# chaeyeongyun/VQ_SEG

Hardware: AMD Instinct MI355X
Metric: train images/sec @512x512 vqreptunet1x1 K=512 (higher is better)
Workload: dtype bf16; 1 GPU; CPS training iteration (2 x vqreptunet1x1, ResNet-50 encoder, K=[0,0,512,512,512], v1 recipe: 6 forwards + 4 backwards + 2 Adam steps) on 512x512x3 images -- BASELINE configs[2] (the metric's configuration): vqreptunet1x1 512x512, K = 512; labelled_per_gpu=32, unlabelled_per_gpu=32, parallelism=dp1, collectives=none (one process), conv_dtype=bf16

## Files before the change

### vq_seg_amd/csrc/loss_kernels.h

```cpp
#pragma once
#include <hip/hip_runtime.h>
#include <stdint.h>

namespace vqseg {

struct ProtoArgs {
    const void* x;
    int bf16;
    const float* proto;
    const long long* labels;
    const unsigned char* keep;
    const float* conf;
    long M;
    int C, K, variant;
    float scale, cos_m, sin_m, th, mm;
    int easy_margin, use_margin;
};

constexpr int PROTO_ROWS_PER_BLOCK = 256;
long proto_blocks(long M);
hipError_t launch_proto_forward(const ProtoArgs& a, double* partial, double* loss, hipStream_t st);
hipError_t launch_proto_backward(const ProtoArgs& a, const float* g_loss, void* gx, float* gproto_partial, float* gproto,
                                 hipStream_t st);

struct DiceArgs {
    const float* logits;
    long sb, sc, sp;
    const long long* target;
    int B, C;
    long HW;
    long long ignore_index;
};
hipError_t launch_softmax_stats(const DiceArgs& a, long long* label, float* entropy, float* top, hipStream_t st);
size_t order_stats_workspace_bytes();
hipError_t launch_order_stats(const float* x, long n, long k, void* workspace, float* out2, hipStream_t st);
hipError_t launch_confusion(const DiceArgs& a, long long* out, hipStream_t st);
constexpr int DICE_PX_PER_BLOCK = 4096;
long dice_blocks(long HW);
hipError_t launch_dice_forward(const DiceArgs& a, double* partial, float* inter, float* sets, float* ce, hipStream_t st);
hipError_t launch_dice_backward(const DiceArgs& a, const float* g_inter, const float* g_sets, const float* g_ce, float* g_logits,
                                hipStream_t st);

struct CombineArgs {
    const float* inter[4]; const float* sets[4]; const float* ce[4];
    float* g_inter[4]; float* g_sets[4]; float* g_ce[4];
    int b[4];
    int n_sup, n_cps, c;
    float cps_weight, ce_weight, eps;
    const float* commit[4]; int n_commit, levels; float commit_weight;
    const double* proto[4]; int n_proto; float proto_weight;
    float* out;
// ... 5 lines not shown
```

### vq_seg_amd/csrc/loss_kernels.hip

```cpp
#include <hip/hip_runtime.h>
#include <stdint.h>

#include "loss_kernels.h"

namespace vqseg {

namespace {

typedef float f32x4 __attribute__((ext_vector_type(4)));
typedef unsigned int u32x4 __attribute__((ext_vector_type(4)));
constexpr int MAXC = 64, MAXK = 4;

template <typename T>
__device__ __forceinline__ void load_row(const T* __restrict__ x, long row, int C, float (&u)[MAXC]) {
    if constexpr (sizeof(T) == 2) {
        const u32x4* p = reinterpret_cast<const u32x4*>(x + row * C);
#pragma unroll
        for (int j = 0; j < MAXC / 8; ++j)
            if (j * 8 < C) {
                const u32x4 v = p[j];
#pragma unroll
                for (int e = 0; e < 4; ++e) {
                    u[j * 8 + 2 * e] = __builtin_bit_cast(float, v[e] << 16);
                    u[j * 8 + 2 * e + 1] = __builtin_bit_cast(float, v[e] & 0xFFFF0000u);
                }
            }
    } else {
        const f32x4* p = reinterpret_cast<const f32x4*>(x + row * C);
#pragma unroll
        for (int j = 0; j < MAXC / 4; ++j)
            if (j * 4 < C) {
                const f32x4 v = p[j];
#pragma unroll
                for (int e = 0; e < 4; ++e) u[j * 4 + e] = v[e];
            }
    }
}

__device__ __forceinline__ float phi_of(float c, const ProtoArgs& a) {
    float inner = 1.0f - c * c;
    inner = inner < 0.0f ? 0.0f : (inner > 1.0f ? 1.0f : inner);
    const float ph = c * a.cos_m - sqrtf(inner) * a.sin_m;
    return a.easy_margin ? (c > 0.0f ? ph : c) : (c > a.th ? ph : c - a.mm);
}
__device__ __forceinline__ float dphi_of(float c, const ProtoArgs& a) {
    const float inner = 1.0f - c * c;
    const float dsine = (inner > 0.0f && inner <= 1.0f) ? -c / sqrtf(inner) : 0.0f;
    const float d = a.cos_m - a.sin_m * dsine;
    return a.easy_margin ? (c > 0.0f ? d : 1.0f) : (c > a.th ? d : 1.0f);
}

struct RowTerms {
    double ll, w;
    double dcos[MAXK];
    float cosv[MAXK];
    float inv_n;
};

__device__ __forceinline__ RowTerms row_terms(const ProtoArgs& a, long row, float n2, const float (&dot)[MAXK], bool want_grad) {
    RowTerms t;
    const float n = fmaxf(sqrtf(n2), 1e-12f);
    t.inv_n = 1.0f / n;
    const int tgt = (int)a.labels[row];
    double z[MAXK], dz[MAXK], oh[MAXK];
#pragma unroll
    for (int c = 0; c < MAXK; ++c)
        if (c < a.K) {
            const float cs = dot[c] * t.inv_n;
            t.cosv[c] = cs;
            if (a.variant == 1) {
                oh[c] = (c == tgt ? 1.0 : 0.0) + 1e-6;
                if (a.use_margin) {
                    z[c] = oh[c] * (double)phi_of(cs, a) + (1.0 - oh[c]) * (double)cs;
                    dz[c] = oh[c] * (double)dphi_of(cs, a) + (1.0 - oh[c]);
                } else {
                    z[c] = (double)cs;
                    dz[c] = 1.0;
                }
            } else {
                oh[c] = c == tgt ? 1.0 : 0.0;
                if (c == tgt) {
                    const float ph = phi_of(cs, a);
                    z[c] = (double)(cs * ph);
                    dz[c] = (double)ph + (double)cs * (double)dphi_of(cs, a);
                } else {
                    z[c] = (double)cs;
                    dz[c] = 1.0;
                }
            }
            z[c] *= (double)a.scale;
            dz[c] *= (double)a.scale;
        }
    double S = 0.0, total = 0.0;
#pragma unroll
    for (int c = 0; c < MAXK; ++c)
        if (c < a.K) {
            S += z[c] * oh[c];
            total += exp(z[c]);
        }
    const double positive = exp(S);
    const double den = total + 1e-7;
    const double q = positive / den + 1e-7;
    t.ll = log(q);
    t.w = a.variant == 1 ? ((a.keep == nullptr || a.keep[row]) ? 1.0 : 0.0) : (a.conf ? (double)a.conf[row] : 1.0);
    if (want_grad) {
#pragma unroll
        for (int c = 0; c < MAXK; ++c)
            if (c < a.K) {
                const double dll_dz = (positive * oh[c] / den - positive * exp(z[c]) / (den * den)) / q;
                t.dcos[c] = dll_dz * dz[c];
            }
    }
    return t;
}

template <typename T>
__global__ __launch_bounds__(256) void proto_fwd_kernel(const ProtoArgs a, double* __restrict__ partial) {
    __shared__ float ps[MAXK * MAXC];
    __shared__ double red[256];
    for (int i = threadIdx.x; i < a.K * a.C; i += 256) ps[i] = a.proto[i];
    __syncthreads();
    const long row = (long)blockIdx.x * PROTO_ROWS_PER_BLOCK + threadIdx.x;
    double v = 0.0;
    if (row < a.M) {
        float u[MAXC];
        load_row<T>(reinterpret_cast<const T*>(a.x), row, a.C, u);
        float n2 = 0.0f, dot[MAXK] = {0.f, 0.f, 0.f, 0.f};
#pragma unroll
        for (int i = 0; i < MAXC; ++i)
            if (i < a.C) {
                n2 = __builtin_fmaf(u[i], u[i], n2);
#pragma unroll
                for (int c = 0; c < MAXK; ++c)
                    if (c < a.K) dot[c] = __builtin_fmaf(u[i], ps[c * a.C + i], dot[c]);
            }
        const RowTerms t = row_terms(a, row, n2, dot, false);
        v = t.ll * t.w;
    }
    red[threadIdx.x] = v;
    __syncthreads();
    for (int m = 128; m >= 1; m >>= 1) {
        if ((int)threadIdx.x < m) red[threadIdx.x] += red[threadIdx.x + m];
        __syncthreads();
    }
    if (threadIdx.x == 0) partial[blockIdx.x] = red[0];
}

__global__ __launch_bounds__(256) void proto_loss_final_kernel(const double* __restrict__ partial, long n_blocks, long M,
                                                               double* __restrict__ loss) {
    __shared__ double red[256];
    double s = 0.0;
    for (long i = threadIdx.x; i < n_blocks; i += 256) s += partial[i];
    red[threadIdx.x] = s;
    __syncthreads();
    for (int m = 128; m >= 1; m >>= 1) {
        if ((int)threadIdx.x < m) red[threadIdx.x] += red[threadIdx.x + m];
        __syncthreads();
    }
    if (threadIdx.x == 0) *loss = -red[0] / (double)M;
}

template <typename T>
__global__ __launch_bounds__(256) void proto_bwd_kernel(const ProtoArgs a, const float* __restrict__ g_loss, T* __restrict__ gx,
                                                        float* __restrict__ gproto_partial, int row_tiles) {
    __shared__ float ps[MAXK * MAXC];
    extern __shared__ float tile[];
    for (int i = threadIdx.x; i < a.K * a.C; i += 256) ps[i] = a.proto[i];
    __syncthreads();
    const int KC = a.K * a.C, G = 256 / KC;
    const int pair = threadIdx.x % KC, grp = threadIdx.x / KC;
    const int pc = pair / a.C, pi = pair % a.C;
    float* rs = tile;
    float* gcs = tile + 256 * (a.C + 1);
    float gacc = 0.0f;
    for (int rt = 0; rt < row_tiles; ++rt) {
    const long row = ((long)blockIdx.x * row_tiles + rt) * PROTO_ROWS_PER_BLOCK + threadIdx.x;
    float u[MAXC];
    float gc[MAXK] = {0.f, 0.f, 0.f, 0.f};
    float inv_n = 0.0f;
    float cosv[MAXK] = {0.f, 0.f, 0.f, 0.f};
    const bool live = row < a.M;
    if (live) {
        load_row<T>(reinterpret_cast<const T*>(a.x), row, a.C, u);
        float n2 = 0.0f, dot[MAXK] = {0.f, 0.f, 0.f, 0.f};
#pragma unroll
        for (int i = 0; i < MAXC; ++i)
            if (i < a.C) {
                n2 = __builtin_fmaf(u[i], u[i], n2);
#pragma unroll
                for (int c = 0; c < MAXK; ++c)
                    if (c < a.K) dot[c] = __builtin_fmaf(u[i], ps[c * a.C + i], dot[c]);
            }
        const RowTerms t = row_terms(a, row, n2, dot, true);
        const double k = -(double)g_loss[0] * t.w / (double)a.M;
        inv_n = t.inv_n;
#pragma unroll
        for (int c = 0; c < MAXK; ++c)
            if (c < a.K) {
                gc[c] = (float)(k * t.dcos[c]);
                cosv[c] = t.cosv[c];
            }
        float gs = 0.0f;
#pragma unroll
        for (int c = 0; c < MAXK; ++c)
            if (c < a.K) gs = __builtin_fmaf(gc[c], cosv[c], gs);
        T* grow = gx + row * a.C;
#pragma unroll
        for (int j = 0; j < MAXC / 8; ++j)
            if (j * 8 < a.C) {
                float o[8];
#pragma unroll
                for (int e = 0; e < 8; ++e) {
                    const int i = j * 8 + e;
                    float acc = -gs * (u[i] * inv_n);
#pragma unroll
                    for (int c = 0; c < MAXK; ++c)
                        if (c < a.K) acc = __builtin_fmaf(gc[c], ps[c * a.C + i], acc);
                    o[e] = acc * inv_n;
                }
                if constexpr (sizeof(T) == 2) {
                    u32x4 v;
#pragma unroll
                    for (int e = 0; e < 4; ++e) {
                        const __bf16 lo = (__bf16)o[2 * e], hi = (__bf16)o[2 * e + 1];
                        v[e] = (unsigned)__builtin_bit_cast(unsigned short, lo) | ((unsigned)__builtin_bit_cast(unsigned short, hi) << 16);
                    }
                    *reinterpret_cast<u32x4*>(grow + j * 8) = v;
                } else {
                    *reinterpret_cast<f32x4*>(grow + j * 8) = f32x4{o[0], o[1], o[2], o[3]};
                    *reinterpret_cast<f32x4*>(grow + j * 8 + 4) = f32x4{o[4], o[5], o[6], o[7]};
                }
            }
    }
    if (gproto_partial) {
#pragma unroll
        for (int i = 0; i < MAXC; ++i)
            if (i < a.C) rs[threadIdx.x * (a.C + 1) + i] = live ? u[i] * inv_n : 0.0f;
#pragma unroll
        for (int c = 0; c < MAXK; ++c) gcs[threadIdx.x * MAXK + c] = gc[c];
        __syncthreads();
        if (grp < G)
            for (int r = grp; r < PROTO_ROWS_PER_BLOCK; r += G) gacc = __builtin_fmaf(gcs[r * MAXK + pc], rs[r * (a.C + 1) + pi], gacc);
        __syncthreads();
    }
    }
    if (gproto_partial) {
        float* part = gcs + 256 * MAXK;
        part[threadIdx.x] = grp < G ? gacc : 0.0f;
        __syncthreads();
        if ((int)threadIdx.x < KC) {
            float s = 0.0f;
            for (int g = 0; g < G; ++g) s += part[g * KC + threadIdx.x];
            gproto_partial[(long)blockIdx.x * KC + threadIdx.x] = s;
        }
    }
}

__global__ __launch_bounds__(256) void proto_gproto_final_kernel(const float* __restrict__ partial, long n_blocks, int n,
                                                                 float* __restrict__ out) {
    __shared__ double red[256];
    const int i = blockIdx.x;
    double s = 0.0;
    for (long b = threadIdx.x; b < n_blocks; b += 256) s += (double)partial[b * n + i];
    red[threadIdx.x] = s;
    __syncthreads();
    for (int m = 128; m >= 1; m >>= 1) {
        if ((int)threadIdx.x < m) red[threadIdx.x] += red[threadIdx.x + m];
        __syncthreads();
    }
    if (threadIdx.x == 0) out[i] = (float)red[0];
}

}

long proto_blocks(long M) { return (M + PROTO_ROWS_PER_BLOCK - 1) / PROTO_ROWS_PER_BLOCK; }

hipError_t launch_proto_forward(const ProtoArgs& a, double* partial, double* loss, hipStream_t st) {
    const long nb = proto_blocks(a.M);
    if (a.bf16) hipLaunchKernelGGL(proto_fwd_kernel<__bf16>, dim3((unsigned)nb), dim3(256), 0, st, a, partial);
    else hipLaunchKernelGGL(proto_fwd_kernel<float>, dim3((unsigned)nb), dim3(256), 0, st, a, partial);
    hipLaunchKernelGGL(proto_loss_final_kernel, dim3(1), dim3(256), 0, st, partial, nb, a.M, loss);
    return hipGetLastError();
}

hipError_t launch_proto_backward(const ProtoArgs& a, const float* g_loss, void* gx, float* gproto_partial, float* gproto,
                                 hipStream_t st) {
    const bool gp = gproto_partial && gproto;
    int row_tiles = 1;
    if (gp) {
        const long want = (proto_blocks(a.M) + 2047) / 2048;
        row_tiles = (int)(want < 1 ? 1 : want);
    }
    const long nb = (proto_blocks(a.M) + row_tiles - 1) / row_tiles;
    const size_t lds = gp ? (size_t)(256 * (a.C + 1) + 256 * MAXK + 256) * sizeof(float) : 0;
    float* gpp = gp ? gproto_partial : nullptr;
    if (a.bf16) hipLaunchKernelGGL(proto_bwd_kernel<__bf16>, dim3((unsigned)nb), dim3(256), lds, st, a, g_loss, (__bf16*)gx, gpp, row_tiles);
    else hipLaunchKernelGGL(proto_bwd_kernel<float>, dim3((unsigned)nb), dim3(256), lds, st, a, g_loss, (float*)gx, gpp, row_tiles);
    if (gp) hipLaunchKernelGGL(proto_gproto_final_kernel, dim3(a.K * a.C), dim3(256), 0, st, gproto_partial, nb, a.K * a.C, gproto);
    return hipGetLastError();
}

namespace {
constexpr int DMAXC = 4;

__device__ __forceinline__ void dice_pixel(const DiceArgs& a, int b, long px, float (&p)[DMAXC], int& tgt, bool& keep, float& nll) {
    const long long t = a.target[(long)b * a.HW + px];
    keep = t != a.ignore_index;
    tgt = keep ? (int)t : 0;
    float z[DMAXC], mx = -__builtin_inff();
#pragma unroll
    for (int c = 0; c < DMAXC; ++c)
        if (c < a.C) {
            z[c] = keep ? a.logits[(long)b * a.sb + c * a.sc + px * a.sp] : 0.0f;
            mx = fmaxf(mx, z[c]);
        }
    float sum = 0.0f;
#pragma unroll
    for (int c = 0; c < DMAXC; ++c)
        if (c < a.C) {
            p[c] = expf(z[c] - mx);
            sum += p[c];
        }
    const float inv = 1.0f / sum;
    float zt = 0.0f;
#pragma unroll
    for (int c = 0; c < DMAXC; ++c)
        if (c < a.C) {
            p[c] *= inv;
            if (c == tgt) zt = z[c];
        }
// ... 423 lines not shown
```

### vq_seg_amd/csrc/nn_abi.hip

```cpp
#include <hip/hip_runtime.h>
#include <stdarg.h>
#include <stdio.h>
#include <string.h>

#include "../../include/vqseg.h"
#include "conv_kernels.h"
#include "vq_kernels.h"
#include "nn_kernels.h"
#include "loss_kernels.h"
#include <math.h>

extern "C" int vqseg_set_error(int code, const char* msg);

namespace {
int bad(const char* msg) { return vqseg_set_error(VQSEG_EINVAL, msg); }
int hipfail(hipError_t e, const char* where) {
    char buf[256];
    snprintf(buf, sizeof(buf), "%s: %s", where, hipGetErrorString(e));
    return vqseg_set_error((int)e, buf);
}
bool a16(const void* p) { return (reinterpret_cast<uintptr_t>(p) & 15u) == 0; }

int conv_rows_per_slot(int cout) { return cout >= 64 ? 64 : 32; }
}
// ... 73 lines not shown
        hipError_t e = vqseg::launch_conv(a, 0, static_cast<hipStream_t>(stream));
        return e == hipSuccess ? 0 : hipfail(e, "conv kernel (split-3)");
    }
    return conv2d_impl(x, x2, c1, w_hi, w_lo, y, nullptr, scale, shift, res, relu, n, h, w, cin, cout, kh, kw, stride, pad, reflect, 1,
                       ho, wo, precise, stream);
}

int vqseg_conv2d_affine_bits_f(const void* x, const void* w_hi, const float* scale, const float* shift, const void* res,
                               const unsigned char* res_bits, void* y, int n, int h, int w, int cin, int cout, int kh, int kw, int pad,
                               int ho, int wo, void* stream) {
    if (!scale || !shift || !res || !res_bits) return bad("conv2d_affine_bits: null pointer");
    if (!a16(res)) return bad("conv2d_affine_bits: pointers must be 16-byte aligned");
    if (cout % 8) return bad("conv2d_affine_bits: Cout must be a multiple of 8");
    return conv2d_impl(x, nullptr, cin, w_hi, nullptr, y, nullptr, scale, shift, res, 0, n, h, w, cin, cout, kh, kw, 1, pad, 0, 1, ho, wo, 0,
                       stream, res_bits);
}

int vqseg_conv_profile_begin(int capacity) {
    if (capacity <= 0 || capacity > (1 << 20)) return bad("conv_profile_begin: capacity out of range");
    hipError_t e = vqseg::conv_profile_begin(capacity);
    return e == hipSuccess ? 0 : hipfail(e, "conv_profile_begin");
}

int vqseg_conv_profile_collect(int max_records, double* flops_host, int* kind_host, float* ms_host, int* shape_host) {
    if (max_records <= 0 || !flops_host || !kind_host || !ms_host) return bad("conv_profile_collect: bad argument");
    return vqseg::conv_profile_collect(max_records, flops_host, kind_host, ms_host, shape_host);
}

int vqseg_set_option(const char* key, int value) {
    if (!key || value < 0) return bad("set_option: null key or negative value");
    int prev = vqseg::conv_set_option(key, value);
    if (prev < 0) prev = vqseg::vq_set_option(key, value);
    if (prev < 0) prev = vqseg::nn_set_option(key, value);
    return prev < 0 ? bad("set_option: unknown key") : prev;
}

size_t vqseg_conv2d_wgrad_workspace_bytes(int n, int h, int w, int cin, int ho, int wo, int cout, int kh, int kw) {
    if (n <= 0 || cin <= 0 || cout <= 0) return 0;
    vqseg::WgradArgs a{};
    a.N = n; a.H = h; a.W = w; a.Cin = cin; a.Ho = ho; a.Wo = wo; a.Cout = cout; a.KH = kh; a.KW = kw;
    return (size_t)vqseg::wgrad_slabs_max(a) * cout * kh * kw * cin * sizeof(float);
}

int vqseg_conv2d_wgrad2_f(const void* gy, const void* x, const void* x2, int n, const void* gy_b, const void* x_b, const void* x2_b,
                          int n_b, int c1, int h, int w, int cin, int ho, int wo, int cout, int kh, int kw, int stride, int pad,
                          int reflect, int precise, int cin_out, int im2col, int accumulate, void* workspace, size_t workspace_bytes,
                          float* gw, void* stream) {
    if (!gy || !x || !workspace || !gw) return bad("conv2d_wgrad: null pointer");
    if (n <= 0 || n_b < 0) return bad("conv2d_wgrad: bad image count");
    if (n_b > 0 && (!gy_b || !x_b)) return bad("conv2d_wgrad: second source missing");
    const int epc = precise ? 4 : 8;
    if (cin % epc || cout % epc) return bad("conv2d_wgrad: Cin and Cout must be multiples of 4 (f32) / 8 (bf16)");
    if (c1 <= 0 || c1 > cin || (c1 < cin && (!x2 || (n_b > 0 && !x2_b) || c1 % epc || (cin - c1) % epc))) return bad("conv2d_wgrad: bad channel split");
    vqseg::WgradArgs a;
    const int kkh = im2col ? 1 : kh, kkw = im2col ? 1 : kw;
    a.gy = gy; a.x = x; a.x2 = x2; a.C1 = c1; a.partial = static_cast<float*>(workspace);
    a.gy_b = gy_b; a.x_b = x_b; a.x2_b = x2_b; a.Na = n;
    a.N = n + n_b; a.H = h; a.W = w; a.Cin = cin; a.Ho = ho; a.Wo = wo; a.Cout = cout; a.KH = kkh; a.KW = kkw;
    a.stride = stride; a.pad = pad; a.reflect = reflect; a.per_tap_only = im2col;
    const int slabs = vqseg::wgrad_slabs(a, precise);
    if (workspace_bytes < (size_t)slabs * cout * kkh * kkw * cin * sizeof(float)) return vqseg_set_error(VQSEG_ENOSPC, "conv2d_wgrad: workspace too small");
    hipStream_t st = static_cast<hipStream_t>(stream);
    int final_layout = 0;
    hipError_t e = vqseg::launch_wgrad(a, precise, slabs, &final_layout, st);
    if (e != hipSuccess) return hipfail(e, "conv_wgrad_kernel");
    if (final_layout && (cin_out != cin || im2col)) return bad("conv2d_wgrad: internal layout mismatch");
// ... 412 lines not shown
```

### vq_seg_amd/csrc/nn_kernels.hip

```cpp
#include <hip/hip_runtime.h>
#include <limits.h>
#include <stdint.h>
#include <string.h>

#include "nn_kernels.h"
#include "options.h"

namespace vqseg {

typedef float f32x4 __attribute__((ext_vector_type(4)));

template <typename T>
__device__ __forceinline__ float ld(const T* p, long i) { return (float)p[i]; }
template <typename T>
__device__ __forceinline__ void st(T* p, long i, float v) { p[i] = (T)v; }

template <typename T>
struct VecN { static constexpr int N = 16 / sizeof(T); };
typedef unsigned int u32x4 __attribute__((ext_vector_type(4)));

template <typename T>
__device__ __forceinline__ void ldv(const T* p, long i, float (&v)[VecN<T>::N]) {
    const u32x4 raw = *reinterpret_cast<const u32x4*>(p + i);
    if constexpr (sizeof(T) == 4) {
// ... 734 lines not shown
    i0 = (int)s;
    if (i0 > in - 1) i0 = in - 1;
    i1 = i0 + (i0 < in - 1 ? 1 : 0);
    l1 = s - (float)i0;
}

template <typename T, int VC>
__global__ __launch_bounds__(256) void bilinear_fwd_kernel(const T* __restrict__ x, int N, int H, int W, int C, int Ho, int Wo,
                                                           int align, T* __restrict__ y) {
    constexpr int V = VecN<T>::N;
    const int cv = C / VC;
    const long total = (long)N * Ho * Wo * cv;
    for (long i = (long)blockIdx.x * 256 + threadIdx.x; i < total; i += (long)gridDim.x * 256) {
        int c, ow, oh, n;
        split_nhwc(i, cv, Wo, Ho, c, ow, oh, n);
        c *= VC;
        int h0, h1, w0, w1;
        float lh, lw;
        bil_src(oh, H, Ho, align, h0, h1, lh);
        bil_src(ow, W, Wo, align, w0, w1, lw);
        const long b = (long)n * H;
        float v00[V], v01[V], v10[V], v11[V], o[V];
        ldc<T, VC>(x, ((b + h0) * W + w0) * C + c, v00);
        ldc<T, VC>(x, ((b + h0) * W + w1) * C + c, v01);
        ldc<T, VC>(x, ((b + h1) * W + w0) * C + c, v10);
        ldc<T, VC>(x, ((b + h1) * W + w1) * C + c, v11);
#pragma unroll
        for (int e = 0; e < VC; ++e)
            o[e] = bil_mix(v00[e], v01[e], v10[e], v11[e], lh, lw);
        stc<T, VC>(y, (((long)n * Ho + oh) * Wo + ow) * C + c, o);
    }
}

__device__ __forceinline__ void bil_bwd_range(int i, int in, int out, int align, int& lo, int& hi) {
    if (in == 1 || out == 1) {
        lo = 0;
        hi = out - 1;
        return;
    }
    if (align) {
        lo = i > 0 ? ((i - 1) * (out - 1)) / (in - 1) - 1 : 0;
        hi = ((i + 1) * (out - 1) + in - 2) / (in - 1) + 1;
    } else {
        lo = i > 0 ? ((2 * i - 1) * out) / (2 * in) - 1 : 0;
        hi = ((2 * i + 3) * out + 2 * in - 1) / (2 * in);
    }
    if (lo < 0) lo = 0;
    if (hi > out - 1) hi = out - 1;
}

template <typename T, int VC>
__global__ __launch_bounds__(256) void bilinear_bwd_kernel(const T* __restrict__ g, int N, int H, int W, int C, int Ho, int Wo,
                                                           int align, T* __restrict__ gx) {
    constexpr int V = VecN<T>::N;
    const int cv = C / VC;
    const long total = (long)N * H * W * cv;
    for (long i = (long)blockIdx.x * 256 + threadIdx.x; i < total; i += (long)gridDim.x * 256) {
        int c, iw, ih, n;
        split_nhwc(i, cv, W, H, c, iw, ih, n);
        c *= VC;
        int oh_lo, oh_hi, ow_lo, ow_hi;
        bil_bwd_range(ih, H, Ho, align, oh_lo, oh_hi);
        bil_bwd_range(iw, W, Wo, align, ow_lo, ow_hi);
        float acc[V];
#pragma unroll
        for (int e = 0; e < VC; ++e) acc[e] = 0.0f;
        for (int oh = oh_lo; oh <= oh_hi; ++oh) {
            int h0, h1;
            float lh;
            bil_src(oh, H, Ho, align, h0, h1, lh);
            float wh = 0.0f;
            if (h0 == ih) wh += 1.0f - lh;
            if (h1 == ih) wh += lh;
            if (wh == 0.0f) continue;
            for (int ow = ow_lo; ow <= ow_hi; ++ow) {
                int w0, w1;
                float lw;
                bil_src(ow, W, Wo, align, w0, w1, lw);
                float ww = 0.0f;
                if (w0 == iw) ww += 1.0f - lw;
                if (w1 == iw) ww += lw;
                if (ww == 0.0f) continue;
                float gv[V];
                ldc<T, VC>(g, (((long)n * Ho + oh) * Wo + ow) * C + c, gv);
#pragma unroll
                for (int e = 0; e < VC; ++e) acc[e] = __builtin_fmaf(wh * ww, gv[e], acc[e]);
            }
        }
        stc<T, VC>(gx, (((long)n * H + ih) * W + iw) * C + c, acc);
    }
}

__device__ __forceinline__ void up2_src(int o, int in, int& i0, int& i1, float& l1) {
    const int i = o >> 1;
    if (o & 1) {
        i0 = i;
        i1 = i + (i < in - 1 ? 1 : 0);
        l1 = 0.25f;
    } else if (o == 0) {
        i0 = 0;
        i1 = in > 1 ? 1 : 0;
        l1 = 0.0f;
    } else {
        i0 = i - 1;
        i1 = i;
        l1 = 0.75f;
    }
}

template <typename T, int VC>
__global__ __launch_bounds__(256) void bilinear_up2_fwd_kernel(const T* __restrict__ x, int N, int H, int W, int C, int lcv, int lwo, int lho,
                                                               T* __restrict__ y) {
    constexpr int V = VecN<T>::N;
    const int Ho = 2 * H, Wo = 2 * W;
    const long total = ((long)N << (lcv + lwo + lho));
    for (long i = (long)blockIdx.x * 256 + threadIdx.x; i < total; i += (long)gridDim.x * 256) {
        const int c = ((int)i & ((1 << lcv) - 1)) * VC;
        const int ow = (int)(i >> lcv) & (Wo - 1), oh = (int)(i >> (lcv + lwo)) & (Ho - 1), n = (int)(i >> (lcv + lwo + lho));
        int h0, h1, w0, w1;
        float lh, lw;
        up2_src(oh, H, h0, h1, lh);
        up2_src(ow, W, w0, w1, lw);
// ... 658 lines not shown
        for (int a = 0; a < nh; ++a)
            for (int bb = 0; bb < nw; ++bb) {
                if (a == 0 && bb == 0) continue;
                const int pa = hs[a], pb = ws[bb];
                const int q = pa == 0 ? pb : (pa == Hp - 1 ? Wp + pb : (pb == 0 ? 2 * Wp + pa - 1 : 2 * Wp + (Hp - 2) + pa - 1));
                float v[V];
                ldc<T, VC>(ring, ((long)n * rl + q) * C + c, v);
#pragma unroll
                for (int e = 0; e < VC; ++e) acc[e] += v[e];
            }
        stc<T, VC>(gx, o, acc);
    }
}

template <typename TI, typename TO>
__global__ __launch_bounds__(256) void cast_kernel(const TI* __restrict__ x, long n, TO* __restrict__ y) {
    for (long i = (long)blockIdx.x * 256 + threadIdx.x; i < n; i += (long)gridDim.x * 256) y[i] = (TO)(float)x[i];
}

static int g_grid_cap = 8192;
long nn_grid_cap() { return g_grid_cap; }
static inline unsigned grid_for(long work, int per_block = 256, long cap = 0) {
    if (cap == 0) cap = g_grid_cap;
    long b = (work + per_block - 1) / per_block;
    if (b < 1) b = 1;
    if (b > cap) b = cap;
    return (unsigned)b;
}

static int g_debug_skip_small = 0;
static int g_bn_bwd_premask = 1;
static int g_bilinear_up2 = 1;
static int g_im2col_strip = 1;

static const Option NN_OPTIONS[] = {
    {"debug_skip_small", &g_debug_skip_small},
    {"bn_bwd_premask", &g_bn_bwd_premask, OPT_FLAG},
    {"nn_grid_cap", &g_grid_cap, OPT_RANGE_FAIL, 256, INT_MAX},
    {"im2col_strip", &g_im2col_strip, OPT_FLAG},
    {"bilinear_up2", &g_bilinear_up2},
};

int nn_set_option(const char* key, int value) {
    if (key && !strcmp(key, "bilinear_up2") && value > 2) value = 1;
    return apply_option(NN_OPTIONS, key, value);
}

hipError_t launch_bn_finalize(float* partial, long n_slots, int rows_per_slot, long M, int C, const float* gamma,
                              const float* beta, float* run_mean, float* run_var, float momentum, float eps, float* scale,
                              float* shift, float* save_mean, float* save_invstd, long long* num_batches_tracked, int* sync,
                              hipStream_t st_) {
    long spg = 1;
    if (g_debug_skip_small & 1) return hipSuccess;
    if (n_slots > 128) {
        spg = (n_slots + 127) / 128;
        if (spg < 16) spg = 16;
        const long groups = (n_slots + spg - 1) / spg;
        if (sync && groups > 1) {
            hipLaunchKernelGGL(bn_stats_merge_finalize_kernel, dim3((C + 63) / 64, (unsigned)groups), dim3(256), 0, st_, partial, n_slots, spg,
                               rows_per_slot, M, C, gamma, beta, run_mean, run_var, momentum, eps, scale, shift, save_mean, save_invstd,
                               num_batches_tracked, sync);
            return hipGetLastError();
        }
        hipLaunchKernelGGL(bn_stats_merge_kernel, dim3((C + 63) / 64, (unsigned)groups), dim3(256), 0, st_, partial, n_slots, spg,
                           rows_per_slot, M, C);
    }
    hipLaunchKernelGGL(bn_finalize_kernel, dim3((C + 63) / 64), dim3(256), 0, st_, partial, n_slots, spg, rows_per_slot, M, C, gamma,
                       beta, run_mean, run_var, momentum, eps, scale, shift, save_mean, save_invstd, num_batches_tracked);
    return hipGetLastError();
}

hipError_t launch_bn_eval_coeffs(int C, const float* gamma, const float* beta, const float* run_mean, const float* run_var,
                                 float eps, float* scale, float* shift, float* save_mean, float* save_invstd, hipStream_t st_) {
// ... 72 lines not shown
        if (bf16) { CALL_B; } else { CALL_F; } \
    } while (0)

template <typename T, int VC>
static void maxpool_t(int backward, const void* x, const void* g, int N, int H, int W, int C, int Ho, int Wo, void* out,
                      unsigned char* idx, hipStream_t st_) {
    if (!backward)
        hipLaunchKernelGGL((maxpool_fwd_kernel<T, VC>), dim3(grid_for((long)N * Ho * Wo * (C / VC))), dim3(256), 0, st_, (const T*)x, N, H,
                           W, C, Ho, Wo, (T*)out, idx);
    else if (idx)
        hipLaunchKernelGGL((maxpool_bwd_idx_kernel<T, VC>), dim3(grid_for((long)N * H * W * (C / VC))), dim3(256), 0, st_, idx,
                           (const T*)g, N, H, W, C, Ho, Wo, (T*)out, (const T*)(backward == 2 ? x : nullptr));
    else
        hipLaunchKernelGGL((maxpool_bwd_kernel<T, VC>), dim3(grid_for((long)N * H * W * (C / VC))), dim3(256), 0, st_, (const T*)x,
                           (const T*)g, N, H, W, C, Ho, Wo, (T*)out);
}

hipError_t launch_maxpool(int bf16, int backward, const void* x, const void* g, int N, int H, int W, int C, void* out,
                          unsigned char* idx, hipStream_t st_) {
    const int Ho = (H + 2 - 3) / 2 + 1, Wo = (W + 2 - 3) / 2 + 1;
    if (bf16) {
        if (C % 8 == 0) maxpool_t<__bf16, 8>(backward, x, g, N, H, W, C, Ho, Wo, out, idx, st_);
        else maxpool_t<__bf16, 1>(backward, x, g, N, H, W, C, Ho, Wo, out, idx, st_);
    } else {
        if (C % 4 == 0) maxpool_t<float, 4>(backward, x, g, N, H, W, C, Ho, Wo, out, idx, st_);
        else maxpool_t<float, 1>(backward, x, g, N, H, W, C, Ho, Wo, out, idx, st_);
    }
    return hipGetLastError();
}

static int ilog2(int v) { int l = 0; while ((1 << l) < v) ++l; return l; }
static bool is_pow2(int v) { return v > 0 && (v & (v - 1)) == 0; }

template <typename T, int VC>
static void bilinear_t(int backward, const void* src, int N, int H, int W, int C, int Ho, int Wo, int align, void* dst,
                       hipStream_t st_) {
    const int cv = C / VC;
    if (g_bilinear_up2 && VC > 1 && !align && Ho == 2 * H && Wo == 2 * W && is_pow2(cv) && is_pow2(H) && is_pow2(W) &&
        (long)N * Ho * Wo * cv < (1L << 40)) {
        if (!backward)
            hipLaunchKernelGGL((bilinear_up2_fwd_kernel<T, VC>), dim3(grid_for((long)N * Ho * Wo * cv)), dim3(256), 0, st_, (const T*)src, N, H,
                               W, C, ilog2(cv), ilog2(Wo), ilog2(Ho), (T*)dst);
        else if (g_bilinear_up2 == 1 && H >= 4)
            hipLaunchKernelGGL((bilinear_up2_bwd_rows_kernel<T, VC, 4>), dim3(grid_for((long)N * (H / 4) * W * cv)), dim3(256), 0, st_,
                               (const T*)src, N, H, W, C, ilog2(cv), ilog2(W), ilog2(H / 4), (T*)dst);
        else
            hipLaunchKernelGGL((bilinear_up2_bwd_kernel<T, VC>), dim3(grid_for((long)N * H * W * cv)), dim3(256), 0, st_, (const T*)src, N, H, W,
                               C, ilog2(cv), ilog2(W), ilog2(H), (T*)dst);
        return;
    }
    if (!backward)
        hipLaunchKernelGGL((bilinear_fwd_kernel<T, VC>), dim3(grid_for((long)N * Ho * Wo * (C / VC))), dim3(256), 0, st_, (const T*)src, N,
                           H, W, C, Ho, Wo, align, (T*)dst);
    else
        hipLaunchKernelGGL((bilinear_bwd_kernel<T, VC>), dim3(grid_for((long)N * H * W * (C / VC))), dim3(256), 0, st_, (const T*)src, N, H,
                           W, C, Ho, Wo, align, (T*)dst);
}

hipError_t launch_bilinear(int bf16, int backward, const void* src, int N, int H, int W, int C, int Ho, int Wo, int align,
                           void* dst, hipStream_t st_) {
    if (bf16) {
        if (C % 8 == 0) bilinear_t<__bf16, 8>(backward, src, N, H, W, C, Ho, Wo, align, dst, st_);
        else bilinear_t<__bf16, 1>(backward, src, N, H, W, C, Ho, Wo, align, dst, st_);
    } else {
        if (C % 4 == 0) bilinear_t<float, 4>(backward, src, N, H, W, C, Ho, Wo, align, dst, st_);
        else if (C == 3) bilinear_t<float, 3>(backward, src, N, H, W, C, Ho, Wo, align, dst, st_);
        else bilinear_t<float, 1>(backward, src, N, H, W, C, Ho, Wo, align, dst, st_);
    }
    return hipGetLastError();
}

hipError_t launch_head_fwd(int bf16, const void* x, const float* w, long M, int Cin, int Cout, float* y, hipStream_t st_) {
    const unsigned gr = grid_for(M);
    if (bf16 == 2) hipLaunchKernelGGL(head_fwd_kernel<S3Row>, dim3(gr), dim3(256), 0, st_, (const S3Row*)x, w, M, Cin, Cout, y);
    else if (bf16) hipLaunchKernelGGL(head_fwd_kernel<__bf16>, dim3(gr), dim3(256), 0, st_, (const __bf16*)x, w, M, Cin, Cout, y);
    else hipLaunchKernelGGL(head_fwd_kernel<float>, dim3(gr), dim3(256), 0, st_, (const float*)x, w, M, Cin, Cout, y);
    return hipGetLastError();
}

long head_bwd_blocks(long M) { return (M + HEAD_ROWS - 1) / HEAD_ROWS; }

hipError_t launch_head_bwd(int bf16, const void* x, const float* w, const float* g, long M, int Cin, int Cout, void* gx,
                           float* gw, float* partial, const void* gx_add, hipStream_t st_) {
// ... 120 lines not shown
```

Baseline: 441.9 images/sec.

## Specialize proto loss kernels on channel count and add tap-table bilinear kernels

Templates the prototype-loss forward and backward kernels on a compile-time channel count so loops unroll fully, and gives the backward a gproto reduction in which each thread accumulates all K prototypes for one channel using vectorized LDS reads. Separately adds tiled bilinear resize kernels for the non-2x-upsample paths that precompute source offsets and weights (forward) and per-output tap lists (backward) in shared memory. The backward form gathers contributions per input pixel instead of searching for them. Also adds compile-time ablation switches and runtime options for both features. The cost is more kernel instantiations and extra shared-memory setup per tile.

New measurement: 445.0 images/sec (median of 6 runs). No clear change (+0.7%).

```diff
diff --git a/vq_seg_amd/csrc/loss_kernels.h b/vq_seg_amd/csrc/loss_kernels.h
--- a/vq_seg_amd/csrc/loss_kernels.h
+++ b/vq_seg_amd/csrc/loss_kernels.h
@@ -17,6 +17,7 @@
     int easy_margin, use_margin;
 };
 
+int loss_set_option(const char* key, int value);
 constexpr int PROTO_ROWS_PER_BLOCK = 256;
 long proto_blocks(long M);
 hipError_t launch_proto_forward(const ProtoArgs& a, double* partial, double* loss, hipStream_t st);
diff --git a/vq_seg_amd/csrc/loss_kernels.hip b/vq_seg_amd/csrc/loss_kernels.hip
--- a/vq_seg_amd/csrc/loss_kernels.hip
+++ b/vq_seg_amd/csrc/loss_kernels.hip
@@ -2,6 +2,11 @@
 #include <stdint.h>
 
 #include "loss_kernels.h"
+#include "options.h"
+
+#ifndef PROTO_ABL
+#define PROTO_ABL 0
+#endif
 
 namespace vqseg {
 
@@ -49,6 +54,14 @@
     const float d = a.cos_m - a.sin_m * dsine;
     return a.easy_margin ? (c > 0.0f ? d : 1.0f) : (c > a.th ? d : 1.0f);
 }
+
+#if PROTO_ABL & 2
+#define PROTO_EXP(v) ((double)expf((float)(v)))
+#define PROTO_LOG(v) ((double)logf((float)(v)))
+#else
+#define PROTO_EXP(v) exp(v)
+#define PROTO_LOG(v) log(v)
+#endif
 
 struct RowTerms {
     double ll, w;
@@ -96,43 +109,44 @@
     for (int c = 0; c < MAXK; ++c)
         if (c < a.K) {
             S += z[c] * oh[c];
-            total += exp(z[c]);
-        }
-    const double positive = exp(S);
+            total += PROTO_EXP(z[c]);
+        }
+    const double positive = PROTO_EXP(S);
     const double den = total + 1e-7;
     const double q = positive / den + 1e-7;
-    t.ll = log(q);
+    t.ll = PROTO_LOG(q);
     t.w = a.variant == 1 ? ((a.keep == nullptr || a.keep[row]) ? 1.0 : 0.0) : (a.conf ? (double)a.conf[row] : 1.0);
     if (want_grad) {
 #pragma unroll
         for (int c = 0; c < MAXK; ++c)
             if (c < a.K) {
-                const double dll_dz = (positive * oh[c] / den - positive * exp(z[c]) / (den * den)) / q;
+                const double dll_dz = (positive * oh[c] / den - positive * PROTO_EXP(z[c]) / (den * den)) / q;
                 t.dcos[c] = dll_dz * dz[c];
             }
     }
     return t;
 }
 
-template <typename T>
+template <typename T, int CT>
 __global__ __launch_bounds__(256) void proto_fwd_kernel(const ProtoArgs a, double* __restrict__ partial) {
     __shared__ float ps[MAXK * MAXC];
     __shared__ double red[256];
-    for (int i = threadIdx.x; i < a.K * a.C; i += 256) ps[i] = a.proto[i];
+    const int C = CT ? CT : a.C;
+    for (int i = threadIdx.x; i < a.K * C; i += 256) ps[i] = a.proto[i];
     __syncthreads();
     const long row = (long)blockIdx.x * PROTO_ROWS_PER_BLOCK + threadIdx.x;
     double v = 0.0;
     if (row < a.M) {
         float u[MAXC];
-        load_row<T>(reinterpret_cast<const T*>(a.x), row, a.C, u);
+        load_row<T>(reinterpret_cast<const T*>(a.x), row, C, u);
         float n2 = 0.0f, dot[MAXK] = {0.f, 0.f, 0.f, 0.f};
 #pragma unroll
         for (int i = 0; i < MAXC; ++i)
-            if (i < a.C) {
+            if (i < C) {
                 n2 = __builtin_fmaf(u[i], u[i], n2);
 #pragma unroll
                 for (int c = 0; c < MAXK; ++c)
-                    if (c < a.K) dot[c] = __builtin_fmaf(u[i], ps[c * a.C + i], dot[c]);
+                    if (c < a.K) dot[c] = __builtin_fmaf(u[i], ps[c * C + i], dot[c]);
             }
         const RowTerms t = row_terms(a, row, n2, dot, false);
         v = t.ll * t.w;
@@ -160,19 +174,22 @@
     if (threadIdx.x == 0) *loss = -red[0] / (double)M;
 }
 
-template <typename T>
+template <typename T, int CT, bool FAST>
 __global__ __launch_bounds__(256) void proto_bwd_kernel(const ProtoArgs a, const float* __restrict__ g_loss, T* __restrict__ gx,
                                                         float* __restrict__ gproto_partial, int row_tiles) {
     __shared__ float ps[MAXK * MAXC];
     extern __shared__ float tile[];
-    for (int i = threadIdx.x; i < a.K * a.C; i += 256) ps[i] = a.proto[i];
-    __syncthreads();
-    const int KC = a.K * a.C, G = 256 / KC;
+    const int C = CT ? CT : a.C;
+    for (int i = threadIdx.x; i < a.K * C; i += 256) ps[i] = a.proto[i];
+    __syncthreads();
+    const int KC = a.K * C, G = 256 / KC;
     const int pair = threadIdx.x % KC, grp = threadIdx.x / KC;
-    const int pc = pair / a.C, pi = pair % a.C;
+    const int pc = pair / C, pi = pair % C;
+    const int Q = 256 / C, fq = threadIdx.x / C, fi = threadIdx.x % C;
     float* rs = tile;
-    float* gcs = tile + 256 * (a.C + 1);
+    float* gcs = tile + 256 * (C + 1);
     float gacc = 0.0f;
+    float facc[MAXK] = {0.f, 0.f, 0.f, 0.f};
     for (int rt = 0; rt < row_tiles; ++rt) {
     const long row = ((long)blockIdx.x * row_tiles + rt) * PROTO_ROWS_PER_BLOCK + threadIdx.x;
     float u[MAXC];
@@ -181,15 +198,15 @@
     float cosv[MAXK] = {0.f, 0.f, 0.f, 0.f};
     const bool live = row < a.M;
     if (live) {
-        load_row<T>(reinterpret_cast<const T*>(a.x), row, a.C, u);
+        load_row<T>(reinterpret_cast<const T*>(a.x), row, C, u);
         float n2 = 0.0f, dot[MAXK] = {0.f, 0.f, 0.f, 0.f};
 #pragma unroll
         for (int i = 0; i < MAXC; ++i)
-            if (i < a.C) {
+            if (i < C) {
                 n2 = __builtin_fmaf(u[i], u[i], n2);
 #pragma unroll
                 for (int c = 0; c < MAXK; ++c)
-                    if (c < a.K) dot[c] = __builtin_fmaf(u[i], ps[c * a.C + i], dot[c]);
+                    if (c < a.K) dot[c] = __builtin_fmaf(u[i], ps[c * C + i], dot[c]);
             }
         const RowTerms t = row_terms(a, row, n2, dot, true);
         const double k = -(double)g_loss[0] * t.w / (double)a.M;
@@ -204,10 +221,10 @@
 #pragma unroll
         for (int c = 0; c < MAXK; ++c)
             if (c < a.K) gs = __builtin_fmaf(gc[c], cosv[c], gs);
-        T* grow = gx + row * a.C;
+        T* grow = gx + row * C;
 #pragma unroll
         for (int j = 0; j < MAXC / 8; ++j)
-            if (j * 8 < a.C) {
+            if (j * 8 < C && !(PROTO_ABL & 4)) {
                 float o[8];
 #pragma unroll
                 for (int e = 0; e < 8; ++e) {
@@ -215,7 +232,7 @@
                     float acc = -gs * (u[i] * inv_n);
 #pragma unroll
                     for (int c = 0; c < MAXK; ++c)
-                        if (c < a.K) acc = __builtin_fmaf(gc[c], ps[c * a.C + i], acc);
+                        if (c < a.K) acc = __builtin_fmaf(gc[c], ps[c * C + i], acc);
                     o[e] = acc * inv_n;
                 }
                 if constexpr (sizeof(T) == 2) {
@@ -232,26 +249,48 @@
                 }
             }
     }
-    if (gproto_partial) {
+    if (gproto_partial && !(PROTO_ABL & 1)) {
 #pragma unroll
         for (int i = 0; i < MAXC; ++i)
-            if (i < a.C) rs[threadIdx.x * (a.C + 1) + i] = live ? u[i] * inv_n : 0.0f;
+            if (i < C) rs[threadIdx.x * (C + 1) + i] = live ? u[i] * inv_n : 0.0f;
 #pragma unroll
         for (int c = 0; c < MAXK; ++c) gcs[threadIdx.x * MAXK + c] = gc[c];
         __syncthreads();
-        if (grp < G)
-            for (int r = grp; r < PROTO_ROWS_PER_BLOCK; r += G) gacc = __builtin_fmaf(gcs[r * MAXK + pc], rs[r * (a.C + 1) + pi], gacc);
+        if constexpr (FAST) {
+            if (fq < Q)
+                for (int r = fq; r < PROTO_ROWS_PER_BLOCK; r += Q) {
+                    const float rv = rs[r * (C + 1) + fi];
+                    const f32x4 gv = *reinterpret_cast<const f32x4*>(gcs + r * MAXK);
+#pragma unroll
+                    for (int c = 0; c < MAXK; ++c) facc[c] = __builtin_fmaf(gv[c], rv, facc[c]);
+                }
+        } else {
+            if (grp < G)
+                for (int r = grp; r < PROTO_ROWS_PER_BLOCK; r += G) gacc = __builtin_fmaf(gcs[r * MAXK + pc], rs[r * (C + 1) + pi], gacc);
+        }
         __syncthreads();
     }
     }
     if (gproto_partial) {
         float* part = gcs + 256 * MAXK;
-        part[threadIdx.x] = grp < G ? gacc : 0.0f;
-        __syncthreads();
-        if ((int)threadIdx.x < KC) {
-            float s = 0.0f;
-            for (int g = 0; g < G; ++g) s += part[g * KC + threadIdx.x];
-            gproto_partial[(long)blockIdx.x * KC + threadIdx.x] = s;
+        if constexpr (FAST) {
+            part = rs;
+#pragma unroll
+            for (int c = 0; c < MAXK; ++c) part[c * 256 + threadIdx.x] = fq < Q ? facc[c] : 0.0f;
+            __syncthreads();
+            if ((int)threadIdx.x < KC) {
+                float s = 0.0f;
+                for (int q = 0; q < Q; ++q) s += part[pc * 256 + q * C + pi];
+                gproto_partial[(long)blockIdx.x * KC + threadIdx.x] = s;
+            }
+        } else {
+            part[threadIdx.x] = grp < G ? gacc : 0.0f;
+            __syncthreads();
+            if ((int)threadIdx.x < KC) {
+                float s = 0.0f;
+                for (int g = 0; g < G; ++g) s += part[g * KC + threadIdx.x];
+                gproto_partial[(long)blockIdx.x * KC + threadIdx.x] = s;
+            }
         }
     }
 }
@@ -275,10 +314,41 @@
 
 long proto_blocks(long M) { return (M + PROTO_ROWS_PER_BLOCK - 1) / PROTO_ROWS_PER_BLOCK; }
 
+static int g_proto_fast = 1;
+static const Option LOSS_OPTIONS[] = {
+    {"proto_fast", &g_proto_fast, OPT_FLAG},
+};
+int loss_set_option(const char* key, int value) { return apply_option(LOSS_OPTIONS, key, value); }
+
+template <typename T, int CT>
+static void proto_forward_t(const ProtoArgs& a, long nb, double* partial, hipStream_t st) {
+    hipLaunchKernelGGL((proto_fwd_kernel<T, CT>), dim3((unsigned)nb), dim3(256), 0, st, a, partial);
+}
+template <typename T, int CT>
+static void proto_backward_t(const ProtoArgs& a, long nb, size_t lds, const float* g_loss, void* gx, float* gpp, int row_tiles, hipStream_t st) {
+    hipLaunchKernelGGL((proto_bwd_kernel<T, CT, CT != 0>), dim3((unsigned)nb), dim3(256), lds, st, a, g_loss, (T*)gx, gpp, row_tiles);
+}
+#define PROTO_DISPATCH(fn, ...)                                                   \
+    do {                                                                          \
+        const int ct = g_proto_fast ? a.C : 0;                                    \
+        if (a.bf16) {                                                             \
+            if (ct == 8) fn<__bf16, 8>(__VA_ARGS__);                              \
+            else if (ct == 16) fn<__bf16, 16>(__VA_ARGS__);                       \
+            else if (ct == 32) fn<__bf16, 32>(__VA_ARGS__);                       \
+            else if (ct == 64) fn<__bf16, 64>(__VA_ARGS__);                       \
+            else fn<__bf16, 0>(__VA_ARGS__);                                      \
+        } else {                                                                  \
+            if (ct == 8) fn<float, 8>(__VA_ARGS__);                               \
+            else if (ct == 16) fn<float, 16>(__VA_ARGS__);                        \
+            else if (ct == 32) fn<float, 32>(__VA_ARGS__);                        \
+            else if (ct == 64) fn<float, 64>(__VA_ARGS__);                        \
+            else fn<float, 0>(__VA_ARGS__);                                       \
+        }                                                                         \
+    } while (0)
+
 hipError_t launch_proto_forward(const ProtoArgs& a, double* partial, double* loss, hipStream_t st) {
     const long nb = proto_blocks(a.M);
-    if (a.bf16) hipLaunchKernelGGL(proto_fwd_kernel<__bf16>, dim3((unsigned)nb), dim3(256), 0, st, a, partial);
-    else hipLaunchKernelGGL(proto_fwd_kernel<float>, dim3((unsigned)nb), dim3(256), 0, st, a, partial);
+    PROTO_DISPATCH(proto_forward_t, a, nb, partial, st);
     hipLaunchKernelGGL(proto_loss_final_kernel, dim3(1), dim3(256), 0, st, partial, nb, a.M, loss);
     return hipGetLastError();
 }
@@ -294,8 +364,7 @@
     const long nb = (proto_blocks(a.M) + row_tiles - 1) / row_tiles;
     const size_t lds = gp ? (size_t)(256 * (a.C + 1) + 256 * MAXK + 256) * sizeof(float) : 0;
     float* gpp = gp ? gproto_partial : nullptr;
-    if (a.bf16) hipLaunchKernelGGL(proto_bwd_kernel<__bf16>, dim3((unsigned)nb), dim3(256), lds, st, a, g_loss, (__bf16*)gx, gpp, row_tiles);
-    else hipLaunchKernelGGL(proto_bwd_kernel<float>, dim3((unsigned)nb), dim3(256), lds, st, a, g_loss, (float*)gx, gpp, row_tiles);
+    PROTO_DISPATCH(proto_backward_t, a, nb, lds, g_loss, gx, gpp, row_tiles, st);
     if (gp) hipLaunchKernelGGL(proto_gproto_final_kernel, dim3(a.K * a.C), dim3(256), 0, st, gproto_partial, nb, a.K * a.C, gproto);
     return hipGetLastError();
 }
diff --git a/vq_seg_amd/csrc/nn_abi.hip b/vq_seg_amd/csrc/nn_abi.hip
--- a/vq_seg_amd/csrc/nn_abi.hip
+++ b/vq_seg_amd/csrc/nn_abi.hip
@@ -129,6 +129,7 @@
     int prev = vqseg::conv_set_option(key, value);
     if (prev < 0) prev = vqseg::vq_set_option(key, value);
     if (prev < 0) prev = vqseg::nn_set_option(key, value);
+    if (prev < 0) prev = vqseg::loss_set_option(key, value);
     return prev < 0 ? bad("set_option: unknown key") : prev;
 }
 
diff --git a/vq_seg_amd/csrc/nn_kernels.hip b/vq_seg_amd/csrc/nn_kernels.hip
--- a/vq_seg_amd/csrc/nn_kernels.hip
+++ b/vq_seg_amd/csrc/nn_kernels.hip
@@ -790,7 +790,7 @@
     }
 }
 
-__device__ __forceinline__ void bil_bwd_range(int i, int in, int out, int align, int& lo, int& hi) {
+__host__ __device__ __forceinline__ void bil_bwd_range(int i, int in, int out, int align, int& lo, int& hi) {
     if (in == 1 || out == 1) {
         lo = 0;
         hi = out - 1;
@@ -846,6 +846,131 @@
             }
         }
         stc<T, VC>(gx, (((long)n * H + ih) * W + iw) * C + c, acc);
+    }
+}
+
+constexpr int TAPS_FWD_COLS = 512, TAPS_BWD_COLS = 256, TAPS_ROWS = 16, TAPS_MAX_LIST = 24;
+
+template <typename T, int VC>
+__global__ __launch_bounds__(256) void bilinear_taps_fwd_kernel(const T* __restrict__ x, int N, int H, int W, int C, int Ho, int Wo,
+                                                                int align, int th, T* __restrict__ y) {
+    constexpr int V = VecN<T>::N;
+    __shared__ int s_o0[TAPS_FWD_COLS], s_o1[TAPS_FWD_COLS], s_h0[TAPS_ROWS], s_h1[TAPS_ROWS];
+    __shared__ float s_lw[TAPS_FWD_COLS], s_lh[TAPS_ROWS];
+    const int cv = C / VC, J = Wo * cv;
+    const int jt = (J + TAPS_FWD_COLS - 1) / TAPS_FWD_COLS, ht = (Ho + th - 1) / th;
+    const long tiles = (long)N * ht * jt;
+    for (long t = blockIdx.x; t < tiles; t += gridDim.x) {
+        const int j0 = (int)(t % jt) * TAPS_FWD_COLS, r0 = (int)((t / jt) % ht) * th, n = (int)(t / jt / ht);
+        const int nj = J - j0 < TAPS_FWD_COLS ? J - j0 : TAPS_FWD_COLS, nr = Ho - r0 < th ? Ho - r0 : th;
+        __syncthreads();
+        for (int j = threadIdx.x; j < nj; j += 256) {
+            const int ow = (j0 + j) / cv, c = (j0 + j - ow * cv) * VC;
+            int w0, w1;
+            float lw;
+            bil_src(ow, W, Wo, align, w0, w1, lw);
+            s_o0[j] = w0 * C + c;
+            s_o1[j] = w1 * C + c;
+            s_lw[j] = lw;
+        }
+        if ((int)threadIdx.x < nr) {
+            int h0, h1;
+            float lh;
+            bil_src(r0 + threadIdx.x, H, Ho, align, h0, h1, lh);
+            s_h0[threadIdx.x] = h0;
+            s_h1[threadIdx.x] = h1;
+            s_lh[threadIdx.x] = lh;
+        }
+        __syncthreads();
+        for (int r = 0; r < nr; ++r) {
+            const T* x0 = x + ((long)n * H + s_h0[r]) * W * C;
+            const T* x1 = x + ((long)n * H + s_h1[r]) * W * C;
+            T* yr = y + ((long)n * Ho + r0 + r) * Wo * C + (long)j0 * VC;
+            const float lh = s_lh[r];
+            for (int j = threadIdx.x; j < nj; j += 256) {
+                const int o0 = s_o0[j], o1 = s_o1[j];
+                const float lw = s_lw[j];
+                float v00[V], v01[V], v10[V], v11[V], o[V];
+                ldc<T, VC>(x0, o0, v00);
+                ldc<T, VC>(x0, o1, v01);
+                ldc<T, VC>(x1, o0, v10);
+                ldc<T, VC>(x1, o1, v11);
+#pragma unroll
+                for (int e = 0; e < VC; ++e)
+                    o[e] = bil_mix(v00[e], v01[e], v10[e], v11[e], lh, lw);
+                stc<T, VC>(yr, (long)j * VC, o);
+            }
+        }
+    }
+}
+
+__device__ __forceinline__ int bil_bwd_list(int i, int in, int out, int align, int cap, int scale, int add, int stride, int* pos, float* wgt) {
+    int lo, hi, k = 0;
+    bil_bwd_range(i, in, out, align, lo, hi);
+    for (int d = lo; d <= hi; ++d) {
+        int i0, i1;
+        float l1;
+        bil_src(d, in, out, align, i0, i1, l1);
+        float w = 0.0f;
+        if (i0 == i) w += 1.0f - l1;
+        if (i1 == i) w += l1;
+        if (w == 0.0f || k >= cap) continue;
+        pos[k * stride] = d * scale + add;
+        wgt[k * stride] = w;
+        ++k;
+    }
+    return k;
+}
+
+template <typename T, int VC>
+__global__ __launch_bounds__(256) void bilinear_taps_bwd_kernel(const T* __restrict__ g, int N, int H, int W, int C, int Ho, int Wo,
+                                                                int align, int th, int lh_cap, int lw_cap, T* __restrict__ gx) {
+    constexpr int V = VecN<T>::N;
+    extern __shared__ int taps_lds[];
+    int* c_cnt = taps_lds;
+    int* c_pos = c_cnt + TAPS_BWD_COLS;
+    float* c_w = reinterpret_cast<float*>(c_pos + lw_cap * TAPS_BWD_COLS);
+    int* r_cnt = reinterpret_cast<int*>(c_w + lw_cap * TAPS_BWD_COLS);
+    int* r_pos = r_cnt + TAPS_ROWS;
+    float* r_w = reinterpret_cast<float*>(r_pos + TAPS_ROWS * lh_cap);
+    const int cv = C / VC, J = W * cv;
+    const int jt = (J + TAPS_BWD_COLS - 1) / TAPS_BWD_COLS, ht = (H + th - 1) / th;
+    const long tiles = (long)N * ht * jt;
+    for (long t = blockIdx.x; t < tiles; t += gridDim.x) {
+        const int j0 = (int)(t % jt) * TAPS_BWD_COLS, r0 = (int)((t / jt) % ht) * th, n = (int)(t / jt / ht);
+        const int nj = J - j0 < TAPS_BWD_COLS ? J - j0 : TAPS_BWD_COLS, nr = H - r0 < th ? H - r0 : th;
+        __syncthreads();
+        const int j = threadIdx.x;
+        if (j < nj) {
+            const int iw = (j0 + j) / cv, c = (j0 + j - iw * cv) * VC;
+            c_cnt[j] = bil_bwd_list(iw, W, Wo, align, lw_cap, C, c, TAPS_BWD_COLS, c_pos + j, c_w + j);
+        }
+        if (j >= 256 - nr) {
+            const int r = 255 - j;
+            r_cnt[r] = bil_bwd_list(r0 + r, H, Ho, align, lh_cap, 1, 0, 1, r_pos + r * lh_cap, r_w + r * lh_cap);
+        }
+        __syncthreads();
+        if (j < nj) {
+            const int cw = c_cnt[j];
+            for (int r = 0; r < nr; ++r) {
+                const int ch = r_cnt[r];
+                float acc[V];
+#pragma unroll
+                for (int e = 0; e < VC; ++e) acc[e] = 0.0f;
+                for (int a = 0; a < ch; ++a) {
+                    const T* grow = g + ((long)n * Ho + r_pos[r * lh_cap + a]) * Wo * C;
+                    const float wh = r_w[r * lh_cap + a];
+                    for (int b = 0; b < cw; ++b) {
+                        const float ww = c_w[b * TAPS_BWD_COLS + j];
+                        float gv[V];
+                        ldc<T, VC>(grow, c_pos[b * TAPS_BWD_COLS + j], gv);
+#pragma unroll
+                        for (int e = 0; e < VC; ++e) acc[e] = __builtin_fmaf(wh * ww, gv[e], acc[e]);
+                    }
+                }
+                stc<T, VC>(gx + ((long)n * H + r0 + r) * W * C, (long)(j0 + j) * VC, acc);
+            }
+        }
     }
 }
 
@@ -1570,6 +1695,7 @@
 static int g_bn_bwd_premask = 1;
 static int g_bilinear_up2 = 1;
 static int g_im2col_strip = 1;
+static int g_bilinear_taps = 1;
 
 static const Option NN_OPTIONS[] = {
     {"debug_skip_small", &g_debug_skip_small},
@@ -1577,6 +1703,7 @@
     {"nn_grid_cap", &g_grid_cap, OPT_RANGE_FAIL, 256, INT_MAX},
     {"im2col_strip", &g_im2col_strip, OPT_FLAG},
     {"bilinear_up2", &g_bilinear_up2},
+    {"bilinear_taps", &g_bilinear_taps, OPT_RANGE_FAIL, 0, TAPS_ROWS},
 };
 
 int nn_set_option(const char* key, int value) {
@@ -1715,6 +1842,16 @@
 static int ilog2(int v) { int l = 0; while ((1 << l) < v) ++l; return l; }
 static bool is_pow2(int v) { return v > 0 && (v & (v - 1)) == 0; }
 
+static int bil_bwd_list_cap(int in, int out, int align) {
+    int cap = 1;
+    for (int i = 0; i < in; ++i) {
+        int lo, hi;
+        bil_bwd_range(i, in, out, align, lo, hi);
+        if (hi - lo + 1 > cap) cap = hi - lo + 1;
+    }
+    return cap;
+}
+
 template <typename T, int VC>
 static void bilinear_t(int backward, const void* src, int N, int H, int W, int C, int Ho, int Wo, int align, void* dst,
                        hipStream_t st_) {
@@ -1732,6 +1869,24 @@
                                C, ilog2(cv), ilog2(W), ilog2(H), (T*)dst);
         return;
     }
+    if (g_bilinear_taps && (long)(W > Wo ? W : Wo) * C < (1L << 31)) {
+        const int rows = backward ? H : Ho, J = (backward ? W : Wo) * cv, cols = backward ? TAPS_BWD_COLS : TAPS_FWD_COLS;
+        int th = g_bilinear_taps > 1 ? g_bilinear_taps : TAPS_ROWS;
+        while (g_bilinear_taps == 1 && th > 1 && (long)N * ((rows + th - 1) / th) * ((J + cols - 1) / cols) < 2048) th >>= 1;
+        const long tiles = (long)N * ((rows + th - 1) / th) * ((J + cols - 1) / cols);
+        if (!backward) {
+            hipLaunchKernelGGL((bilinear_taps_fwd_kernel<T, VC>), dim3(grid_for(tiles, 1)), dim3(256), 0, st_, (const T*)src, N, H, W, C, Ho, Wo,
+                               align, th, (T*)dst);
+            return;
+        }
+        const int lh = bil_bwd_list_cap(H, Ho, align), lw = bil_bwd_list_cap(W, Wo, align);
+        if (lh <= TAPS_MAX_LIST && lw <= TAPS_MAX_LIST) {
+            const size_t lds = sizeof(int) * (size_t)(TAPS_BWD_COLS * (1 + 2 * lw) + TAPS_ROWS * (1 + 2 * lh));
+            hipLaunchKernelGGL((bilinear_taps_bwd_kernel<T, VC>), dim3(grid_for(tiles, 1)), dim3(256), lds, st_, (const T*)src, N, H, W, C, Ho, Wo,
+                               align, th, lh, lw, (T*)dst);
+            return;
+        }
+    }
     if (!backward)
         hipLaunchKernelGGL((bilinear_fwd_kernel<T, VC>), dim3(grid_for((long)N * Ho * Wo * (C / VC))), dim3(256), 0, st_, (const T*)src, N,
                            H, W, C, Ho, Wo, align, (T*)dst);
```
